# bmorris3/frei

Hardware: AMD Instinct MI355X
Metric: lambda-bin*layer flux updates/sec at 60 layers x 500k lambda (higher is better)
Workload: dtype f64; 1 GPU; C3/C4: 60 layers x 500000 lambda, 8 species (H2O/CO/CO2/CH4/Na/K + H2-H2/H2-He CIA), 16 T-nodes, 1 step = 1 T-P iteration (emit+absorb); n_layers=60, n_lambda=500000, n_species=8, n_T=16, parallelism=lambda-shard x1

## Files before the change

frei_amd/csrc/frei_device.h:

```cpp
#pragma once
#include <hip/hip_runtime.h>

#include <algorithm>
#include <cstdint>
#include <string>

namespace frei {

constexpr double kH = 6.62607015e-27;
constexpr double kC = 29979245800.0;
constexpr double kHC = kH * kC;
constexpr double kKB = 1.380649e-16;
constexpr double kMP = 1.67262192369e-24;
constexpr double kMbarDefault = 2.4 * kMP;
constexpr double kSigmaSB = 5.6703744191844314e-05;
constexpr double kPi = 3.141592653589793;

constexpr int kEmit = 0;
constexpr int kAbsorb = 1;
constexpr int kBlock = 256;
constexpr int kMaxLayers = 1024;

__host__ __device__ inline int step_layer(int dir, int k, int nL) {
  return dir == kEmit ? k + 1 : nL - 2 - k;
}
__host__ __device__ inline int layer_step(int dir, int i, int nL) {
  const int k = dir == kEmit ? i - 1 : nL - 2 - i;
  return (k >= 0 && k < nL - 1) ? k : -1;
}

struct StepP {
  double iT1, iT2;
  double dm;
  int32_t layer;
  int32_t top;
  int64_t pad;
};

constexpr int kMaxFastS = 8;
struct FastStep {
  double iT1, iT2, dm;
  int32_t layer, top;
  double wlo[kMaxFastS], whi[kMaxFastS], mmr[kMaxFastS];
  int64_t off[kMaxFastS];
};

struct FastStepS {
  double iT1, iT2, dm, wlo, whi;
  int64_t off;
  int32_t layer, top;
  double mmr[kMaxFastS];
};
static_assert(sizeof(FastStepS) % sizeof(double) == 0, "FastStepS is staged as doubles");

struct TermP {
  const double* row[4];
  double w[4];
  double mmr;
  double x1, dx;
  int32_t nrow;
  int32_t pad;
};

struct SpecMeta {
  const double* tab;
  int64_t n_lam;
  int32_t n_p, n_T;
  int32_t t_off;
  int32_t one_T;
};

struct PMeta {
  int32_t p_lo, p_hi;
  double wp_lo, wp_hi;
  double x1, dx;
  int32_t oob;
  int32_t pad;
};

__host__ __device__ inline void bracket(const double* g, int n, double x, int& i, double& y,
                                        int& oob) {
  int lo = 0, hi = n;
  while (lo < hi) {
    const int mid = (lo + hi) >> 1;
    if (g[mid] < x) lo = mid + 1; else hi = mid;
  }
  i = lo - 1;
  if (i < 0) i = 0;
  if (i > n - 2) i = n - 2;
  y = (x - g[i]) / (g[i + 1] - g[i]);
  oob = (x < g[0] || x > g[n - 1]) ? 1 : 0;
}

__host__ __device__ inline TermP make_term(const SpecMeta& sm, const PMeta& pm,
                                           const double* tnodes, const int32_t* tperm,
                                           double mmr, double T, int fast) {
  TermP t;
  for (int r = 0; r < 4; ++r) { t.row[r] = sm.tab; t.w[r] = 0.0; }
  t.mmr = mmr;
  t.x1 = 0.0;
  t.dx = 1.0;
  t.nrow = 0;
  t.pad = 0;
  const int64_t rowlen = sm.n_lam;
  if (sm.one_T) {
    if (pm.oob) return t;
    const int tp = tperm[sm.t_off];
    t.row[0] = sm.tab + ((int64_t)pm.p_lo * sm.n_T + tp) * rowlen;
    t.row[1] = sm.tab + ((int64_t)pm.p_hi * sm.n_T + tp) * rowlen;
    t.x1 = pm.x1;
    t.dx = pm.dx;
    t.nrow = -1;
    return t;
  }
  int it, oobT;
  double yt;
  bracket(tnodes + sm.t_off, sm.n_T, T, it, yt, oobT);
  if (pm.oob || oobT) {
    if (fast) t.nrow = 2;
    return t;
  }
  const int tlo = tperm[sm.t_off + it], thi = tperm[sm.t_off + it + 1];
  const int pr[2] = {pm.p_lo, pm.p_hi};
  const double wp[2] = {pm.wp_lo, pm.wp_hi};
  const int tr[2] = {tlo, thi};
  const double wt[2] = {1.0 - yt, yt};
  int n = 0;
  for (int a = 0; a < 2; ++a) {
    if (wp[a] == 0.0) continue;
    for (int b = 0; b < 2; ++b) {
      t.row[n] = sm.tab + ((int64_t)pr[a] * sm.n_T + tr[b]) * rowlen;
      t.w[n] = (1.0 * wp[a]) * wt[b];
      ++n;
    }
  }
  t.nrow = n;
  return t;
}

__host__ __device__ inline void fast_term(const SpecMeta& sm, const PMeta& pm,
                                          const double* tnodes, double T, int64_t& off,
                                          double& wlo, double& whi) {
  int it, oobT;
  double yt;
  bracket(tnodes + sm.t_off, sm.n_T, T, it, yt, oobT);
  off = 0;
  wlo = whi = 0.0;
  if (pm.oob || oobT) return;
  const int prow = (pm.wp_lo != 0.0) ? pm.p_lo : pm.p_hi;
  const double wp = (pm.wp_lo != 0.0) ? pm.wp_lo : pm.wp_hi;
  off = ((int64_t)prow * sm.n_T + it) * sm.n_lam;
  wlo = (1.0 * wp) * (1.0 - yt);
  whi = (1.0 * wp) * yt;
}

struct AtmStride {
  int64_t layers;
  int64_t steps;
  int64_t fb;
  int64_t hist;
  int64_t flux;
  int64_t tab;
  int64_t part;
  int64_t ftoa;
  const double* g;
};

struct ChemArgs {
  const double* tab;
  const double* T;
  const int32_t* pj;
  const double* pz;
  int n_T, n_p;
  const int32_t* atm_tab;
  int64_t tab_stride;
};

__host__ __device__ inline void chem_bracket(const double* g, int n, double x, int& i,
                                             double& y) {
  i = 0;
  y = 0.0;
  if (n < 2) return;
  const double xc = x < g[0] ? g[0] : (x > g[n - 1] ? g[n - 1] : x);
  int lo = 0, hi = n - 2;
  while (lo < hi) {
    const int mid = (lo + hi + 1) >> 1;
    if (g[mid] <= xc) lo = mid; else hi = mid - 1;
  }
  i = lo;
  y = (xc - g[i]) / (g[i + 1] - g[i]);
}

__host__ __device__ inline double chem_mmr_at(const ChemArgs& c, int s, int j, double z,
                                              double T) {
  int it;
  double y;
  chem_bracket(c.T, c.n_T, T, it, y);
  const double* v = c.tab + ((int64_t)s * c.n_T + it) * c.n_p;
  auto row = [&](const double* r) { return c.n_p > 1 ? r[j] * (1.0 - z) + r[j + 1] * z : r[0]; };
  const double a = row(v);
  return c.n_T > 1 ? a * (1.0 - y) + row(v + c.n_p) * y : a;
}

struct SetupArgs {
  ChemArgs chem;
  int n_layers, n_species, fast;
  int n_tnodes;
  double* T;
  const double* p;
  double p_top2, g;
  const SpecMeta* spec;
  const PMeta* pmeta;
  const double* tnodes;
  const int32_t* tperm;
  const double* mmr;
  StepP* steps;
  TermP* terms;
  FastStep* fsteps;
  FastStepS* ssteps;
  int shared;
  AtmStride bs;
  int32_t* kvalid;
  int64_t kpitch;
};

struct FastArgs {
  int64_t n_lam;
  int64_t pitch;
  int n_steps, force;
  int live_only;
  const double *c1, *hcl, *sig, *wtr, *ftoa;
  const double* tab[kMaxFastS];
  const FastStep* steps;
  const FastStepS* ssteps;
  double* F_up;
  double* F_down;
  double* dtaus;
  double* part;
  const int* conv;
  AtmStride bs;
  int n_atm;
  int red_rows;
  int unit_mmr;
  int rec_on;
  SetupArgs rec;
  int min_lds;
  const unsigned long long* ch_epoch;
  unsigned long long ch_val;
  int ch_can_conv;
  long long ch_timeout;
  int* ch_err;
  double* poison;
  const double* ktab[kMaxFastS];
  const double* kmmr;
  int kS, kNL;
  double* tail_part;
};
constexpr unsigned long long kPoisonT = 0xFFF4F4F4F4F4F4F4ull;

struct SweepArgs {
  int64_t n_lam;
  int n_steps, n_species, force;
  int live_only;
  const double *c1, *hcl, *sig, *wtr, *ftoa;
  const StepP* steps;
  const TermP* terms;
  double* F_up;
  double* F_down;
  double* dtaus;
  double* part;
  const int* conv;
};

struct P2PPush {
  double* const* peers;
  int nranks, rank;
  int64_t n;
  uint64_t seq;
};
struct P2PWait {
  const double* mbox;
  int nranks;
  int64_t n;
  uint64_t seq;
  int64_t timeout_ticks;
  int* err;
  unsigned long long* wait_ticks;
};
__host__ __device__ inline int64_t mbox_val(int par, int r, int R, int64_t n) {
// ... 159 lines not shown
```

frei_amd/csrc/frei_kernels.hip:

```cpp
#include <type_traits>
#include <unordered_map>

#include "frei_device.h"
#include "frei_math.h"

namespace frei {

template <auto V, auto... Rest, typename F>
static void pick(decltype(V) v, F&& f) {
  if constexpr (sizeof...(Rest) == 0) {
    f(std::integral_constant<decltype(V), V>{});
  } else {
    if (v == V) f(std::integral_constant<decltype(V), V>{});
    else pick<Rest...>(v, f);
  }
}

static void lds_optin(const void* kernel, size_t lds) {
  if (lds <= 65536) return;
  static std::unordered_map<const void*, size_t> optin;
  size_t& have = optin[kernel];
  if (lds > have) {
    (void)hipFuncSetAttribute(kernel, hipFuncAttributeMaxDynamicSharedMemorySize, (int)lds);
    have = lds;
// ... 1653 lines not shown
    for (int i = 0; i < G; ++i) stn[i] = stale(0, i);
    PT_STAMP(DIR, bx, wv, -1, 0);
    for (int ph = 0; ph <= nph; ++ph) {
      if (ph >= 1) {
        const int q = ph - 1;
        double stc[G];
#pragma unroll
        for (int i = 0; i < G; ++i) stc[i] = stn[i];
#pragma unroll
        for (int i = 0; i < G; ++i) stn[i] = stale(ph, i);
        double rv[G][kPipeNV];
        read_ring(q, rv);
#pragma unroll
        for (int i = 0; i < G; ++i) step(q, i, stc[i], rv[i]);
      }
      PT_STAMP(DIR, bx, wv, ph, 0);
      __syncthreads();
      PT_STAMP(DIR, bx, wv, ph, 1);
    }
  }
  TRACE_MARK(2);
  if constexpr (!TL) {
    __syncthreads();
    for (int idx = tid; idx < ns * 4; idx += 256 * NC) {
      double s = red[idx];
      for (int w = 1; w < NC; ++w) s += red[(int64_t)w * ns * 4 + idx];
      part[part_at(idx, bx, nbx, ns * 4)] = s;
    }
  }
  TRACE_PUT(CH ? 50 + NC : TL ? 60 + NC : 20 + NC);
}

template <int DIR, int NC, int M, int PF>
__global__ __launch_bounds__(256 * NC) __attribute__((amdgpu_waves_per_eu(4)))
void sweep_pipe_kernel(FastArgs a, const FastStepS* __restrict__ ss, double* __restrict__ Fu,
                       double* __restrict__ Fd, double* __restrict__ part,
                       double* __restrict__ dtaus) {
  extern __shared__ double lds[];
  sweep_pipe_body<DIR, NC, M, PF, false>(a, ss, Fu, Fd, part, dtaus, lds, blockIdx.x, gridDim.x);
}

void launch_sweep_pipe(int dir, int NC, int PF, const FastArgs& a, int nblocks,
                       hipStream_t st) {
  pick<kEmit, kAbsorb>(dir, [&](auto D) {
    pick<4, 2, 1>(NC, [&](auto nc) {
      pick<2, 1>(PF, [&](auto pf) {
        launch_lds(sweep_pipe_kernel<D(), nc(), 2, pf()>,
                   dim3(nblocks, a.n_atm > 1 ? a.n_atm : 1), dim3(256 * nc()),
                   pipe_lds_bytes(nc(), 2, a.n_steps), st, a, a.ssteps, a.F_up, a.F_down, a.part,
                   a.dtaus);
      });
    });
  });
}

size_t pipe_lds_bytes(int NC, int M, int ns) {
  return (size_t)pipe_lds_doubles(NC, M, ns) * sizeof(double);
}

__device__ __forceinline__ void p2p_push_values(const P2PPush& p, int64_t idx, const double* v,
                                                int nv) {
  const int par = (int)(p.seq & 1);
  for (int r = 0; r < p.nranks; ++r) {
    uint64_t* dst = reinterpret_cast<uint64_t*>(p.peers[r] + mbox_val(par, p.rank, p.nranks, p.n));
    for (int k = 0; k < nv; ++k)
      __hip_atomic_store(dst + idx + k, __builtin_bit_cast(uint64_t, v[k]), __ATOMIC_RELAXED,
                         __HIP_MEMORY_SCOPE_SYSTEM);
  }
  __builtin_amdgcn_fence(__ATOMIC_RELEASE, "");
  asm volatile("s_waitcnt vmcnt(0)" ::: "memory");
  for (int r = 0; r < p.nranks; ++r) {
    uint64_t* fl = reinterpret_cast<uint64_t*>(p.peers[r]) + mbox_flag(par, p.rank, p.nranks, p.n);
    for (int k = 0; k < nv; ++k)
      __hip_atomic_store(fl + idx + k, p.seq, __ATOMIC_RELAXED, __HIP_MEMORY_SCOPE_SYSTEM);
  }
}

__device__ __forceinline__ void p2p_wait(const P2PWait& w, int r, int64_t idx, long long t0) {
  const int par = (int)(w.seq & 1);
  const uint64_t* fl =
      reinterpret_cast<const uint64_t*>(w.mbox) + mbox_flag(par, r, w.nranks, w.n) + idx;
  while (__hip_atomic_load(fl, __ATOMIC_RELAXED, __HIP_MEMORY_SCOPE_SYSTEM) != w.seq) {
    if (wall_clock64() - t0 > w.timeout_ticks ||
        __hip_atomic_load(w.err, __ATOMIC_RELAXED, __HIP_MEMORY_SCOPE_AGENT)) {
      __hip_atomic_store(w.err, 1, __ATOMIC_RELAXED, __HIP_MEMORY_SCOPE_AGENT);
      break;
    }
    __builtin_amdgcn_s_sleep(1);
  }
}

__device__ __forceinline__ void p2p_acquire() { __builtin_amdgcn_fence(__ATOMIC_ACQUIRE, ""); }

__device__ __forceinline__ double p2p_value(const P2PWait& w, int r, int64_t idx) {
  const int par = (int)(w.seq & 1);
  const uint64_t* vp =
      reinterpret_cast<const uint64_t*>(w.mbox + mbox_val(par, r, w.nranks, w.n)) + idx;
  return __builtin_bit_cast(double,
                            __hip_atomic_load(vp, __ATOMIC_RELAXED, __HIP_MEMORY_SCOPE_SYSTEM));
}

__global__ void p2p_handshake_kernel(P2PPush push, P2PWait wait) {
  if (threadIdx.x != 0) return;
  const double one = 1.0;
  p2p_push_values(push, 0, &one, 1);
  const long long t0 = wall_clock64();
  for (int r = 0; r < wait.nranks; ++r) p2p_wait(wait, r, 0, t0);
  p2p_acquire();
}

void launch_p2p_handshake(const P2PPush& push, const P2PWait& wait, hipStream_t st) {
  hipLaunchKernelGGL(p2p_handshake_kernel, dim3(1), dim3(64), 0, st, push, wait);
}

constexpr int kRedThreads = 256;
constexpr int kRedWaves = kRedThreads / 64;

__global__ __launch_bounds__(kRedThreads) void reduce_kernel(const double* __restrict__ part,
                                                     int nblocks, double* __restrict__ Fb,
                                                     const int* conv, int force,
                                                     int64_t part_stride, int64_t fb_stride,
                                                     P2PPush push) {
  part += blockIdx.y * part_stride;
  Fb += blockIdx.y * fb_stride;
  conv += blockIdx.y;
  if (!force && *conv) return;
  __shared__ double sh[kRedWaves];
  const int ns4 = gridDim.x;
  double acc = 0.0;
  for (int b = threadIdx.x; b < nblocks; b += kRedThreads)
    acc += part[part_at(blockIdx.x, b, nblocks, ns4)];
  acc = butterfly_sum(acc, threadIdx.x & 63);
  if ((threadIdx.x & 63) == 0) sh[threadIdx.x >> 6] = acc;
  __syncthreads();
  if (threadIdx.x == 0) {
    double v = sh[0];
    for (int w = 1; w < kRedWaves; ++w) v += sh[w];
    if (push.peers) p2p_push_values(push, blockIdx.x, &v, 1);
    else Fb[blockIdx.x] = v;
  }
}

__global__ void log_ratio_kernel(const double* __restrict__ p, double p_top2, int nL,
                                 double* __restrict__ lnp) {
  const int l = blockIdx.x * blockDim.x + threadIdx.x;
  if (l < nL) lnp[l] = log(p[l] / (l == nL - 1 ? p_top2 : p[l + 1]));
}

void launch_log_ratio(const double* p, double p_top2, int nL, double* lnp, hipStream_t st) {
  hipLaunchKernelGGL(log_ratio_kernel, dim3((nL + 255) / 256), dim3(256), 0, st, p, p_top2,
                     nL, lnp);
}

__device__ __forceinline__ void step_s_core(const SetupArgs& u, const double* T, const double* P,
                                            const double* tnodes, const SpecMeta& sm,
                                            const PMeta& pm, int dir, int k, FastStepS& f) {
  const int nL = u.n_layers;
  const int i = step_layer(dir, k, nL);
  const int top = (dir == kEmit && i == nL - 1) ? 1 : 0;
  f.layer = i;
  f.top = top;
  f.iT1 = 1.0 / T[i];
  f.iT2 = top ? f.iT1 : 1.0 / T[i + 1];
  const double p2 = top ? u.p_top2 : P[i + 1];
  f.dm = (P[i] - p2) / u.g;
  int64_t off;
  double wlo, whi;
  fast_term(sm, pm, tnodes, T[i], off, wlo, whi);
  f.off = off;
  f.wlo = wlo;
  f.whi = whi;
}
__device__ void setup_sweep(const SetupArgs& u, const double* T, const double* P,
                            const double* tnodes, const SpecMeta* spec, const PMeta* pmeta,
                            const double* mmr, int dir, int kb, int ke, int tid, int nthr,
                            int mstride, int mbase) {
  const int nS = u.n_species;
  const int nL = u.n_layers;
  auto MI = [&](int s, int i) { return (int64_t)s * mstride + (i - mbase); };
  auto MMR = [&](int s, int i) {
    return u.chem.tab ? chem_mmr_at(u.chem, s, u.chem.pj[i], u.chem.pz[i], T[i])
                      : mmr[MI(s, i)];
  };
  if (u.fast && u.shared) {
    for (int k = kb + tid; k < ke; k += nthr) {
      const int i = step_layer(dir, k, nL);
      FastStepS* f = u.ssteps + k;
      step_s_core(u, T, P, tnodes, spec[0], pmeta[MI(0, i)], dir, k, *f);
      for (int s = 0; s < kMaxFastS; ++s) f->mmr[s] = s < nS ? MMR(s, i) : 0.0;
    }
    return;
  }
  if (u.fast) {
    for (int k = kb + tid; k < ke; k += nthr) {
      const int i = step_layer(dir, k, nL);
      FastStep* f = u.fsteps + k;
      const int top = (dir == kEmit && i == nL - 1) ? 1 : 0;
      f->layer = i;
      f->top = top;
      f->iT1 = 1.0 / T[i];
      f->iT2 = top ? f->iT1 : 1.0 / T[i + 1];
      const double p2 = top ? u.p_top2 : P[i + 1];
      f->dm = (P[i] - p2) / u.g;
    }
    for (int idx = tid; idx < (ke - kb) * kMaxFastS; idx += nthr) {
      const int k = kb + idx / kMaxFastS, s = idx % kMaxFastS;
      FastStep* f = u.fsteps + k;
      if (s >= nS) {
        if (!(u.kvalid && s == 1)) f->off[s] = 0;
        f->wlo[s] = f->whi[s] = f->mmr[s] = 0.0;
        continue;
      }
      const int i = step_layer(dir, k, nL);
      int64_t off;
      double wlo, whi;
      fast_term(spec[s], pmeta[MI(s, i)], tnodes, T[i], off, wlo, whi);
      f->off[s] = off;
      f->wlo[s] = wlo;
      f->whi[s] = whi;
      f->mmr[s] = MMR(s, i);
      if (u.kvalid && s == 0) {
        int64_t mask = 0;
        if (wlo != 0.0 || whi != 0.0) {
          const int64_t r = off / u.kpitch;
          mask = (u.kvalid[r] ? 0 : 1) | (u.kvalid[r + 1] ? 0 : 2);
        }
        f->off[1] = mask;
      }
    }
    return;
  }
  for (int k = kb + tid; k < ke; k += nthr) {
    const int i = step_layer(dir, k, nL);
    StepP sp;
    sp.layer = i;
    sp.top = (dir == kEmit && i == nL - 1) ? 1 : 0;
    sp.iT1 = 1.0 / T[i];
    sp.iT2 = sp.top ? sp.iT1 : 1.0 / T[i + 1];
    const double p2 = sp.top ? u.p_top2 : P[i + 1];
    sp.dm = (P[i] - p2) / u.g;
    sp.pad = 0;
    u.steps[k] = sp;
  }
  for (int idx = tid; idx < (ke - kb) * nS; idx += nthr) {
    const int k = kb + idx / nS, s = idx % nS;
    const int i = step_layer(dir, k, nL);
    u.terms[(int64_t)k * nS + s] = make_term(spec[s], pmeta[MI(s, i)], tnodes, u.tperm, MMR(s, i),
                             T[i], u.fast);
  }
}

__device__ inline void atm_view(SetupArgs& u, int m) {
  u.T += m * u.bs.layers;
  u.steps += m * u.bs.steps;
  u.fsteps += m * u.bs.steps;
  u.ssteps += m * u.bs.steps;
  if (u.bs.g) u.g = u.bs.g[m];
  if (u.chem.atm_tab) u.chem.tab += u.chem.atm_tab[m] * u.chem.tab_stride;
}

__device__ inline void atm_view(UpdateArgs& a, int m) {
  atm_view(a.su, m);
  const AtmStride& b = a.su.bs;
  a.Fb += m * b.fb;
  a.Tb += m * b.layers;
  a.Ta += m * b.layers;
  a.hist += m * b.hist;
  a.flips += m * b.layers;
  a.prev_sign += m * b.layers;
  a.ndiff += m * b.layers;
  a.iter += m;
  a.conv += m;
  if (a.dT_out) a.dT_out += m * b.layers;
  if (a.bol_out) a.bol_out += m * b.layers * 4;
}

__global__ void setup_kernel(SetupArgs u, int dir) {
  atm_view(u, blockIdx.x);
  setup_sweep(u, u.T, u.p, u.tnodes, u.spec, u.pmeta, u.mmr, dir, 0, u.n_layers - 1,
              threadIdx.x, blockDim.x, u.n_layers, 0);
}

struct LayerPre {
  double dz, cp, dF_conv, dt_rad, dt_conv, rho0, cp0;
  bool conv;
};

__device__ __forceinline__ LayerPre layer_pre(double T1, double T2, double p1, double p2,
                                              double lnp, double g, double m_bar,
                                              double alpha) {
  LayerPre r;
  r.dz = (kKB * T1) / (m_bar * g) * lnp;
  r.cp = (2 + 5) / (2 * m_bar) * kKB;
  const double rho = ((p1 - p2) / g) / r.dz;
  const double dg = (T1 - T2) / r.dz - g / r.cp;
  r.conv = dg > 0;
  r.dF_conv = 0.0;
  r.dt_conv = 0.0;
  if (r.conv) {
    const double lmix = alpha * kKB * T1 / (m_bar * g);
    r.dF_conv = rho * r.cp * (lmix * lmix) * sqrt(g / T1) * pow(dg, 1.5);
    r.dt_conv = sqrt(T1 / g / dg);
  }
  r.dt_rad = r.cp * p1 / kSigmaSB / g / pow(T1, 3.0);
  const double m0 = kMbarDefault;
  const double dz0 = (kKB * T1) / (m0 * g) * lnp;
  r.rho0 = ((p1 - p2) / g) / dz0;
  r.cp0 = (2 + 5) / (2 * m0) * kKB;
  return r;
}

__device__ __forceinline__ double layer_dT_post(const double* Fb, const LayerPre& r) {
  const double dF_rad = (Fb[0] - Fb[1]) - (Fb[2] - Fb[3]);
  const double div = (dF_rad + r.dF_conv) / r.dz;
  const double x = div * r.dz;
  const double f = (x != 0) ? 1e5 / pow(fabs(x), 0.9) : 1.0;
  const double dt = r.conv ? f * fmin(r.dt_rad, r.dt_conv) : f * r.dt_rad;
  return 1 / r.rho0 / r.cp0 * div * dt;
}

__device__ double layer_dT(const double* Fb, double T1, double T2, double p1, double p2,
                           double lnp, double g, double m_bar, double alpha) {
  return layer_dT_post(Fb, layer_pre(T1, T2, p1, p2, lnp, g, m_bar, alpha));
}


__global__ __launch_bounds__(256) void update_kernel(UpdateArgs a) {
  atm_view(a, blockIdx.x);
  if (!a.force && *a.conv) return;
  extern __shared__ __attribute__((aligned(16))) double sh[];
  __shared__ int all_conv;
  const int nL = a.su.n_layers;
  const int ns = nL - 1;
  const int dir = a.dir;
  const int S = a.su.n_species;
  const int ntn = a.su.n_tnodes;
  double* sT = sh;
  double* sdT = sT + nL;
  double* sP = sdT + nL;
  double* sTb = sP + nL;
  double* sTa = sTb + nL;
  double* sLn = sTa + nL;
  double* sTn = sLn + nL;
  double* sFb = sTn + ntn;
  int* sFl = reinterpret_cast<int*>(sFb + ns * 4);
  int* sPv = sFl + nL;
  int* sNd = sPv + nL;
  const bool meta = a.meta_in_lds;
  char* mb = reinterpret_cast<char*>(sh) + (((reinterpret_cast<char*>(sNd + nL) -
                                              reinterpret_cast<char*>(sh)) + 15) & ~15);
  PMeta* sPm = reinterpret_cast<PMeta*>(mb);
  double* sMm = reinterpret_cast<double*>(sPm + (meta ? S * nL : 0));
  SpecMeta* sSp = reinterpret_cast<SpecMeta*>(sMm + (meta ? S * nL : 0));
  if (threadIdx.x == 0) all_conv = 1;
  for (int l = threadIdx.x; l < nL; l += blockDim.x) {
    sT[l] = a.su.T[l];
    sdT[l] = 0.0;
    sP[l] = a.su.p[l];
    sLn[l] = a.lnp[l];
    if (a.track) {
      sTb[l] = a.Tb[l];
      sTa[l] = a.Ta[l];
      sFl[l] = a.flips[l];
      sPv[l] = a.prev_sign[l];
      sNd[l] = a.ndiff[l];
    }
  }
  for (int q = threadIdx.x; q < ntn; q += blockDim.x) sTn[q] = a.su.tnodes[q];
  if (a.p2p.mbox) {
    const long long t0 = wall_clock64();
    for (int q = threadIdx.x; q < ns * 4; q += blockDim.x)
      for (int r = 0; r < a.p2p.nranks; ++r) p2p_wait(a.p2p, r, q, t0);
    p2p_acquire();
    for (int q = threadIdx.x; q < ns * 4; q += blockDim.x) {
      double v = p2p_value(a.p2p, 0, q);
      for (int r = 1; r < a.p2p.nranks; ++r) v += p2p_value(a.p2p, r, q);
      sFb[q] = v;
    }
    __syncthreads();
    if (threadIdx.x == 0 && a.p2p.wait_ticks)
      atomicAdd(a.p2p.wait_ticks, (unsigned long long)(wall_clock64() - t0));
  } else {
    for (int q = threadIdx.x; q < ns * 4; q += blockDim.x) {
      double v = a.Fb[q];
      for (int r = 1; r < a.nranks; ++r) v += a.Fb[(int64_t)r * ns * 4 + q];
      sFb[q] = v;
    }
  }
  if (meta) {
    for (int q = threadIdx.x; q < S * nL; q += blockDim.x) {
      sPm[q] = a.su.pmeta[q];
      sMm[q] = a.su.mmr[q];
    }
    for (int q = threadIdx.x; q < S; q += blockDim.x) sSp[q] = a.su.spec[q];
  }
  __syncthreads();
  for (int k = threadIdx.x; k < ns; k += blockDim.x) {
    const int i = step_layer(dir, k, nL);
    const double* Fb = sFb + k * 4;
    if (a.bol_out)
      for (int q = 0; q < 4; ++q) a.bol_out[(int64_t)i * 4 + q] = Fb[q];
    const bool top = (dir == kEmit && i == nL - 1);
    const double T1 = sT[i];
    const double T2 = top ? T1 : sT[i + 1];
    const double p2 = top ? a.su.p_top2 : sP[i + 1];
    sdT[i] = layer_dT(Fb, T1, T2, sP[i], p2, sLn[i], a.su.g, a.m_bar, a.alpha);
  }
  __syncthreads();
  const int it = *a.iter;
  for (int l = threadIdx.x; l < nL; l += blockDim.x) {
    const double dT = sdT[l];
    const double Tnew = sT[l] - dT;
    if (a.dT_out) a.dT_out[l] = dT;
    if (a.track) {
      if (dir == kEmit) {
        a.Tb[l] = Tnew;
      } else {
        const double Tb = sTb[l];
        if (it < a.hist_cap) {
          a.hist[((int64_t)it * 2 + 0) * nL + l] = Tb;
          a.hist[((int64_t)it * 2 + 1) * nL + l] = Tnew;
        }
        int flips = sFl[l], prev = sPv[l], nd = sNd[l];
        const double d0 = Tb - sTa[l], d1 = Tnew - Tb;
        for (int q = (it > 0 ? 0 : 1); q < 2; ++q) {
          const double d = q == 0 ? d0 : d1;
          const int sgn = (d > 0) - (d < 0);
          if (nd > 0 && sgn != prev) ++flips;
          prev = sgn;
          ++nd;
        }
        a.flips[l] = flips;
        a.prev_sign[l] = prev;
        a.ndiff[l] = nd;
        a.Ta[l] = Tnew;
        const bool c = (flips > a.n_zero_crossings) || (fabs(dT) < a.convergence_dT);
        if (!c) atomicAnd(&all_conv, 0);
      }
    }
    a.su.T[l] = Tnew;
    sT[l] = Tnew;
  }
  __syncthreads();
  if (threadIdx.x == 0 && a.track && dir == kAbsorb) {
    *a.iter = it + 1;
    if (all_conv && a.stop_on_conv) *a.conv = 1;
  }
  if (a.next_dir >= 0)
    setup_sweep(a.su, sT, sP, sTn, meta ? sSp : a.su.spec, meta ? sPm : a.su.pmeta,
                meta ? sMm : a.su.mmr, a.next_dir, 0, ns, threadIdx.x, blockDim.x, nL, 0);
}

__device__ __forceinline__ void publish_T(const UpdateArgs& a, int l, double T, int conv0,
                                          bool c) {
  if (a.epoch) {
    __hip_atomic_store(reinterpret_cast<unsigned long long*>(a.T_out) + l,
                       __builtin_bit_cast(unsigned long long, T), __ATOMIC_RELAXED,
                       __HIP_MEMORY_SCOPE_AGENT);
    __hip_atomic_store(a.epoch + l,
                       (a.epoch_val << 2) | (conv0 ? 2ull : 0ull) | (c ? 1ull : 0ull),
                       __ATOMIC_RELAXED, __HIP_MEMORY_SCOPE_AGENT);
  } else {
    a.T_out[l] = T;
  }
}
__device__ __forceinline__ void update_arrive(const UpdateArgs& a, int nU, int it, bool nc1) {
  if (!(a.track && a.dir == kAbsorb)) return;
  const unsigned old = __hip_atomic_fetch_add(a.done, 1u + (nc1 ? 65536u : 0u),
                                              __ATOMIC_RELAXED, __HIP_MEMORY_SCOPE_AGENT);
  if ((old & 0xffffu) != (unsigned)nU - 1) return;
  const unsigned nc = (old >> 16) + (nc1 ? 1u : 0u);
  *a.iter = it + 1;
  if (nc == 0 && a.stop_on_conv) *a.conv = 1;
  __hip_atomic_store(a.done, 0u, __ATOMIC_RELAXED, __HIP_MEMORY_SCOPE_AGENT);
}

template <int U = 1>
__device__ void update_fused_body(const UpdateArgs& a, int lr, int nU, int tid, int h,
                                  double* sh) {
  TRACE_DECL;
  const int nL = a.su.n_layers;
  const bool on = lr < nL;
  const int l = on ? lr : nL - 1;
  const int dir = a.dir;
  const double* Tin = a.su.T;
  double* sTn = sh;
  double* sP = sTn + nL;
  double* sNodes = sP + nL;
  __shared__ double wsum_[4][kRedWaves][8];
  __shared__ double tot_[4][8];
  __shared__ PMeta sPm_[4][kMaxFastS];
  __shared__ SpecMeta sSp_[4][kMaxFastS];
  __shared__ double sMm_[4][kMaxFastS];
  auto& wsum = wsum_[h];
  double* tot = tot_[h];
  PMeta* sPm = sPm_[h];
  SpecMeta* sSp = sSp_[h];
  double* sMm = sMm_[h];
  const int k0 = layer_step(dir, l, nL);
  const int k1 = l + 1 < nL ? layer_step(dir, l + 1, nL) : -1;
  const int kn = a.next_dir >= 0 ? layer_step(a.next_dir, l, nL) : -1;
  const int S = a.su.n_species;
  const bool stage = S <= kMaxFastS;
  const int conv = *a.conv;
  const int it = *a.iter;
  const int ntn = a.su.n_tnodes;
  const double rNode = a.su.tnodes[tid < ntn ? tid : ntn - 1];
  const int li = min(l + (tid & 1), nL - 1);
  const int li1 = min(li + 1, nL - 1);
  const int kd = (tid & 1) ? k1 : k0;
  const bool top = (dir == kEmit && li == nL - 1);
  const double T1 = Tin[li];
  const double rT2 = Tin[li1];
  const double p1 = a.su.p[li];
  const double rp2 = a.su.p[li1];
  const double lnp = a.lnp[li];
  const double Tb = a.Tb[l], Ta = a.Ta[l];
  int flips = a.flips[l], prev = a.prev_sign[l], nd = a.ndiff[l];
  const int sm = min(max(tid - 64, 0), S - 1);
  const PMeta rPm = a.su.pmeta[(int64_t)sm * nL + l];
  const SpecMeta rSp = a.su.spec[sm];
  const double rMm = a.su.mmr[(int64_t)sm * nL + l];
  const double T2 = top ? T1 : rT2;
  const double p2 = top ? a.su.p_top2 : rp2;
  const double Tl = T1;
  LayerPre pre{};
  if (tid < 2 && kd >= 0) pre = layer_pre(T1, T2, p1, p2, lnp, a.su.g, a.m_bar, a.alpha);
  if (k0 >= 0 || k1 >= 0) {
    const double* pj[8];
    for (int j = 0; j < 8; ++j) {
      const int k = (j < 4) ? (k0 >= 0 ? k0 : k1) : (k1 >= 0 ? k1 : k0);
      pj[j] = a.part + part_at(k * 4 + (j & 3), 0, a.nblocks, 4 * (nL - 1));
    }
    const int64_t bs = part_at(0, 1, a.nblocks, 4 * (nL - 1));
    double acc[8];
    for (int j = 0; j < 8; ++j) acc[j] = 0.0;
    constexpr int kU = U;
    const int nb = a.nblocks;
    if constexpr (U == 1) {
#pragma unroll 2
      for (int b = tid; b < nb; b += kRedThreads)
        for (int j = 0; j < 8; ++j) acc[j] += pj[j][b * bs];
    } else
    for (int b0 = tid; b0 < nb; b0 += kU * kRedThreads) {
      double v[kU][8];
#pragma unroll
      for (int u = 0; u < kU; ++u) {
        const int b = min(b0 + u * kRedThreads, nb - 1);
#pragma unroll
        for (int j = 0; j < 8; ++j) v[u][j] = pj[j][b * bs];
      }
#pragma unroll
      for (int u = 0; u < kU; ++u)
        if (b0 + u * kRedThreads < nb)
#pragma unroll
          for (int j = 0; j < 8; ++j) acc[j] += v[u][j];
    }
    for (int j = 0; j < 8; ++j)
      acc[j] = butterfly_sum(acc[j], tid & 63);
    if ((tid & 63) == 0)
      for (int j = 0; j < 8; ++j) wsum[tid >> 6][j] = acc[j];
  }
  if (!a.force && conv) {
    if (tid == 0 && on) publish_T(a, l, Tl, conv, true);
    return;
  }
  if (tid < ntn) sNodes[tid] = rNode;
  for (int q = tid + kRedThreads; q < ntn; q += kRedThreads) sNodes[q] = a.su.tnodes[q];
  if (kn >= 0) {
    const int s = tid - 64;
    if (stage && s >= 0 && s < S) {
      sPm[s] = rPm;
      sSp[s] = rSp;
      sMm[s] = rMm;
    }
    if (tid < 2 && l + tid < nL) sP[l + tid] = p1;
    if (tid == 1 && l + 1 < nL) sTn[l + 1] = T1;
  }
  __syncthreads();
  TRACE_MARK(1);
  if (tid < 8) {
    double t = wsum[0][tid];
    for (int w = 1; w < kRedWaves; ++w) t += wsum[w][tid];
    tot[tid] = t;
  }
  __syncthreads();
  const long long t0 = wall_clock64();
  if (a.p2p.mbox && tid == 64 && k0 >= 0 && on)
    p2p_push_values(a.push, (int64_t)k0 * 4, tot, 4);
  if (tid < 64) {
    double v = 0.0;
    const int k = tid < 4 ? k0 : k1;
    if (tid < 8 && k >= 0) {
      v = tot[tid];
      if (a.p2p.mbox) {
        const double own = v;
        const int64_t idx = (int64_t)k * 4 + (tid & 3);
        for (int r = 0; r < a.p2p.nranks; ++r)
          if (r != a.push.rank) p2p_wait(a.p2p, r, idx, t0);
        p2p_acquire();
        for (int r = 0; r < a.p2p.nranks; ++r) {
          const double x = (r == a.push.rank) ? own : p2p_value(a.p2p, r, idx);
          v = (r == 0) ? x : v + x;
        }
      }
    }
    const int base = (tid & 1) * 4;
    double F[4];
    for (int q = 0; q < 4; ++q) F[q] = __shfl(v, base + q, 64);
    if (tid < 4 && k0 >= 0 && a.bol_out && on) a.bol_out[(int64_t)l * 4 + tid] = v;
    if (tid == 0 && lr == 0 && a.p2p.mbox && a.p2p.wait_ticks)
      atomicAdd(a.p2p.wait_ticks, (unsigned long long)(wall_clock64() - t0));
    double d = 0.0;
    if (tid < 2 && kd >= 0) {
      d = layer_dT_post(F, pre);
      sTn[li] = T1 - d;
    }
    if (tid == 0 && on) {
      const double dT = d;
      const double Tnew = Tl - dT;
      if (a.dT_out) a.dT_out[l] = dT;
      bool c = true;
      if (a.track) {
        if (dir == kEmit) {
          a.Tb[l] = Tnew;
        } else {
          if (it < a.hist_cap) {
            a.hist[((int64_t)it * 2 + 0) * nL + l] = Tb;
            a.hist[((int64_t)it * 2 + 1) * nL + l] = Tnew;
          }
          const double d0 = Tb - Ta, d1 = Tnew - Tb;
          for (int q = (it > 0 ? 0 : 1); q < 2; ++q) {
            const double dd = q == 0 ? d0 : d1;
            const int sgn = (dd > 0) - (dd < 0);
            if (nd > 0 && sgn != prev) ++flips;
            prev = sgn;
            ++nd;
          }
          a.flips[l] = flips;
          a.prev_sign[l] = prev;
          a.ndiff[l] = nd;
          a.Ta[l] = Tnew;
          c = (flips > a.n_zero_crossings) || (fabs(dT) < a.convergence_dT);
        }
      }
      publish_T(a, l, Tnew, conv, c);
      if (kd < 0) sTn[l] = Tnew;
      update_arrive(a, nU, it, !c);
    }
  }
  TRACE_MARK(2);
  __syncthreads();
  if (a.su.kvalid && tid == 64 && on && k0 >= 0) {
    int64_t off;
    double wlo, whi;
    fast_term(rSp, rPm, sNodes, Tl, off, wlo, whi);
    if (wlo != 0.0 || whi != 0.0) {
      const int64_t r = off / a.su.kpitch;
      a.su.kvalid[r] = 1;
      a.su.kvalid[r + 1] = 1;
    }
  }
  if (kn >= 0 && tid >= 64 && on) {
    if (stage)
      setup_sweep(a.su, sTn, sP, sNodes, sSp, sPm, sMm, a.next_dir, kn, kn + 1, tid - 64,
                  kRedThreads - 64, 1, l);
    else
      setup_sweep(a.su, sTn, sP, sNodes, a.su.spec, a.su.pmeta, a.su.mmr, a.next_dir, kn,
                  kn + 1, tid - 64, kRedThreads - 64, nL, 0);
  }
  TRACE_PUT(30);
}

__device__ __forceinline__ void update_shadow(const UpdateArgs& a) {
  if (!a.force && *a.conv) return;
  __syncthreads();
  __syncthreads();
  __syncthreads();
}

__global__ __launch_bounds__(kRedThreads) void update_fused_kernel(UpdateArgs a) {
  extern __shared__ __attribute__((aligned(16))) double sh[];
  update_fused_body<8>(a, blockIdx.x, gridDim.x, threadIdx.x, 0, sh);
}

template <int DIR, int Q, int NW>
__global__ __launch_bounds__(64 * NW) void sweep_chain_kernel(
    FastArgs a, UpdateArgs u, const FastStepS* __restrict__ ss, double* __restrict__ Fu,
    double* __restrict__ Fd, double* __restrict__ part, double* __restrict__ dtaus) {
  static_assert(kRedThreads == 256, "update halves of 256 threads");
  extern __shared__ double red[];
  const int nL = u.su.n_layers;
  constexpr int kHalves = NW / 4;
  const int nU = (nL + kHalves - 1) / kHalves;
  if ((int)blockIdx.x < nU) {
    const int h = threadIdx.x >> 8;
    update_fused_body(u, blockIdx.x * kHalves + h, nL, threadIdx.x & 255, h,
                      red + (int64_t)h * (2 * nL + u.su.n_tnodes));
    return;
  }
  sweep_group_body<DIR, Q, NW, true>(a, ss, Fu, Fd, part, dtaus, red, blockIdx.x - nU,
                                     gridDim.x - nU);
}

template <int DIR, int PF>
__global__ __launch_bounds__(1024) __attribute__((amdgpu_waves_per_eu(4)))
void sweep_pipe_chain_kernel(FastArgs a, UpdateArgs u, const FastStepS* __restrict__ ss,
                             double* __restrict__ Fu, double* __restrict__ Fd,
                             double* __restrict__ part, double* __restrict__ dtaus) {
  static_assert(kRedThreads == 256, "update parts of 256 threads");
  extern __shared__ double lds[];
  const int nL = u.su.n_layers;
  if ((int)blockIdx.x < nL) {
    if (threadIdx.x < 256) update_fused_body(u, blockIdx.x, nL, threadIdx.x, 0, lds);
    else update_shadow(u);
    return;
  }
  sweep_pipe_body<DIR, 4, 2, PF, true>(a, ss, Fu, Fd, part, dtaus, lds, blockIdx.x - nL,
                                       gridDim.x - nL);
}

void launch_sweep_pipe_chain(int dir, int PF, const FastArgs& a, const UpdateArgs& u,
                             int nblocks, hipStream_t st) {
  const int nL = u.su.n_layers;
  const size_t shm = std::max(pipe_lds_bytes(4, 2, a.n_steps),
                              (size_t)(2 * nL + u.su.n_tnodes) * sizeof(double));
  pick<kEmit, kAbsorb>(dir, [&](auto D) {
    pick<2, 1>(PF, [&](auto pf) {
      launch_lds(sweep_pipe_chain_kernel<D(), pf()>, dim3(nL + nblocks), dim3(1024), shm, st, a,
                 u, a.ssteps, a.F_up, a.F_down, a.part, a.dtaus);
    });
  });
}

struct TailIn {
  double *T, *p, *Tb, *Ta, *mmr, *nodes;
  int *flips, *prev, *nd;
  PMeta* pm;
  LayerPre* pre;
};
__host__ __device__ inline size_t tail_in_bytes(int nL, int ntn) {
  return (size_t)nL * (sizeof(PMeta) + sizeof(LayerPre)) + (size_t)(5 * nL + ntn) * sizeof(double) +
         (size_t)3 * nL * sizeof(int);
}
__device__ __forceinline__ TailIn tail_in_layout(double* lds, int nL, int ntn) {
  TailIn t;
  t.pre = reinterpret_cast<LayerPre*>(lds);
  t.pm = reinterpret_cast<PMeta*>(t.pre + nL);
  double* d = reinterpret_cast<double*>(t.pm + nL);
  t.T = d;
  t.p = d + nL;
  t.Tb = d + 2 * nL;
  t.Ta = d + 3 * nL;
  t.mmr = d + 4 * nL;
  t.nodes = d + 5 * nL;
  int* q = reinterpret_cast<int*>(t.nodes + ntn);
  t.flips = q;
  t.prev = q + nL;
  t.nd = q + 2 * nL;
  return t;
}

#ifdef FREI_TRACE
__shared__ unsigned long long g_tail_done[4];
__shared__ unsigned g_tail_pass[4];
#endif
__device__ __forceinline__ void tail_update_slot(const UpdateArgs& a, int lr, int tid, int h,
                                                 double (&wsum)[kRedWaves][8],
                                                 const TailIn& in, int conv, int it) {
  TRACE_DECL;
  const int nL = a.su.n_layers;
  const bool on = lr < nL;
  const int l = on ? lr : nL - 1;
  const int dir = a.dir;
  const int k0 = layer_step(dir, l, nL);
  const int k1 = l + 1 < nL ? layer_step(dir, l + 1, nL) : -1;
  const bool skip = !a.force && conv;
  const bool sums = !skip && (k0 >= 0 || k1 >= 0);
  const int nb = a.nblocks;
  if (sums) {
    const double* pj[8];
    for (int j = 0; j < 8; ++j) {
      const int k = (j < 4) ? (k0 >= 0 ? k0 : k1) : (k1 >= 0 ? k1 : k0);
      pj[j] = a.part + (int64_t)(k * 4 + (j & 3)) * nb;
    }
    const int b = min(tid, nb - 1);
    unsigned long long x[8];
    auto load_all = [&]() {
      bool m = false;
#pragma unroll
      for (int j = 0; j < 8; ++j) {
        x[j] = __hip_atomic_load((const gu64*)(pj[j] + b), __ATOMIC_RELAXED, __HIP_MEMORY_SCOPE_AGENT);
        m |= x[j] == kPoisonT;
      }
      return m;
    };
    bool miss = load_all();
#ifdef FREI_TRACE
    int passes = 1;
#endif
    if (__any(miss)) {
      const long long t0 = wall_clock64();
      do {
        __builtin_amdgcn_s_sleep(1);
        miss = load_all();
#ifdef FREI_TRACE
        ++passes;
#endif
        const int e = __hip_atomic_load(a.poll_err, __ATOMIC_RELAXED, __HIP_MEMORY_SCOPE_AGENT);
        if (__any(miss) && (e || wall_clock64() - t0 > a.poll_timeout)) {
          if (!e) __hip_atomic_store(a.poll_err, 3, __ATOMIC_RELAXED, __HIP_MEMORY_SCOPE_AGENT);
          break;
        }
      } while (__any(miss));
    }
#ifdef FREI_TRACE
    atomicMax(&g_tail_done[h], (unsigned long long)wall_clock64());
    atomicMax(&g_tail_pass[h], (unsigned)passes);
#endif
    double acc[8];
    for (int j = 0; j < 8; ++j) acc[j] = tid < nb ? 0.0 + __builtin_bit_cast(double, x[j]) : 0.0;
    for (int j = 0; j < 8; ++j) acc[j] = butterfly_sum(acc[j], tid & 63);
    if ((tid & 63) == 0)
      for (int j = 0; j < 8; ++j) wsum[tid >> 6][j] = acc[j];
  }
  __syncthreads();
  TRACE_MARK(2);
#ifdef FREI_TRACE
  if (sums) {
    unsigned long long dm = 0;
    unsigned pm = 0;
    for (int q = 0; q < 4; ++q) dm = max(dm, g_tail_done[q]), pm = max(pm, g_tail_pass[q]);
    tr_[1] = (long long)(dm & ((1ull << 40) - 1)) | ((long long)pm << 40);
  }
  __syncthreads();
  if (tid == 0) g_tail_done[h] = 0, g_tail_pass[h] = 0;
// ... 634 lines not shown
      smm[q] = a.mmr[((int64_t)(m0 + m) * S + s) * a.n_layers + l];
    }
    __syncthreads();
    if (live)
      for (int m = 0; m < nm; ++m) {
        const double* mm = smm + m * S;
        dbl2 acc = mm[0] * v[0];
#pragma unroll
        for (int s = 1; s < S; ++s) acc = acc + mm[s] * v[s];
        *reinterpret_cast<dbl2*>(a.eff + (int64_t)(m0 + m) * a.tab_stride + at) = acc;
      }
  }
}

void launch_contract_batch_valu(const double* const* tabs, int S, const double* mmr,
                                const int32_t* prow, int n_layers, int n_T, int64_t pitch,
                                int n_atm, int64_t tab_stride, double* eff, hipStream_t st) {
  ContractBatchArgs a{};
  for (int s = 0; s < S && s < kMaxFastS; ++s) a.tab[s] = tabs[s];
  a.mmr = mmr;
  a.prow = prow;
  a.eff = eff;
  a.S = S;
  a.n_layers = n_layers;
  a.n_T = n_T;
  a.n_atm = n_atm;
  a.pitch = pitch;
  a.tab_stride = tab_stride;
  const int64_t ncol = (int64_t)n_T * pitch;
  dim3 grid((unsigned)((ncol / 2 + 255) / 256), (unsigned)n_layers);
  switch (S) {
#define K7V(n) case n: hipLaunchKernelGGL(contract_batch_valu_kernel<n>, grid, dim3(256), 0, st, a); break;
    K7V(1) K7V(2) K7V(3) K7V(4) K7V(5) K7V(6) K7V(7)
    default: hipLaunchKernelGGL(contract_batch_valu_kernel<8>, grid, dim3(256), 0, st, a);
#undef K7V
  }
}

void launch_contract_batch(const double* const* tabs, int S, const double* mmr,
                           const int32_t* prow, int n_layers, int n_T, int64_t pitch,
                           int n_atm, int64_t tab_stride, double* eff, hipStream_t st) {
  ContractBatchArgs a{};
  for (int s = 0; s < S && s < kMaxFastS; ++s) a.tab[s] = tabs[s];
  a.mmr = mmr;
  a.prow = prow;
  a.eff = eff;
  a.S = S;
  a.n_layers = n_layers;
  a.n_T = n_T;
  a.n_atm = n_atm;
  a.pitch = pitch;
  a.tab_stride = tab_stride;
  const int64_t ncol = (int64_t)n_T * pitch;
  dim3 grid((unsigned)((ncol + 4 * kK7Cols - 1) / (4 * kK7Cols)), (unsigned)n_layers);
  switch (S) {
#define K7M(n) case n: hipLaunchKernelGGL(contract_batch_kernel<n>, grid, dim3(256), 0, st, a); break;
    K7M(1) K7M(2) K7M(3) K7M(4) K7M(5) K7M(6) K7M(7)
    default: hipLaunchKernelGGL(contract_batch_kernel<8>, grid, dim3(256), 0, st, a);
#undef K7M
  }
}

__global__ void fill_kernel(double* x, int64_t n, double v) {
  for (int64_t idx = (int64_t)blockIdx.x * blockDim.x + threadIdx.x; idx < n;
       idx += (int64_t)gridDim.x * blockDim.x)
    x[idx] = v;
}

void launch_sweep(int dir, const SweepArgs& a, int nblocks, hipStream_t st) {
  const size_t shm = (size_t)(kBlock / 64) * a.n_steps * 4 * sizeof(double);
  pick<kEmit, kAbsorb>(dir, [&](auto D) {
    launch_lds(sweep_kernel<D()>, dim3(nblocks), dim3(kBlock), shm, st, a);
  });
}

void launch_sweep_fast(int dir, int S, int depth, int pf, bool nan_check, bool shared,
                       const FastArgs& a, int nblocks, hipStream_t st) {
  const bool one = S == 1 && !nan_check;
  const bool mm1 = one && a.unit_mmr;
  int PD = depth >= 2 ? 2 : 1, PF = 0;
  if (mm1 && pf > depth && depth >= 2) {
    PD = fast_pd(depth);
    PF = fast_pf_or_0(pf);
  } else if (mm1 && depth == 1 && pf == 2) {
    PF = 2;
  } else if (one && depth >= 4) {
    PD = 4;
  }
  pick<kEmit, kAbsorb>(dir, [&](auto D) {
    pick<true, false>(shared, [&](auto SH) {
      auto go = [&](auto s, auto pd, auto nanchk, auto m1, auto f) {
        const size_t shm = SH() ? lds_steps_bytes(a)
                                : (size_t)red_lds_doubles(a.red_rows, a.n_steps) * sizeof(double);
        launch_lds(sweep_fast_kernel<D(), s(), pd(), nanchk(), SH(), m1(), f() ? f() : pd()>,
                   dim3(nblocks, a.n_atm > 1 ? a.n_atm : 1), dim3(kBlock), with_min_lds(a, shm),
                   st, a, a.steps, a.ssteps, a.F_up, a.F_down, a.part, a.dtaus);
      };
      constexpr std::integral_constant<int, 1> k1{};
      constexpr std::integral_constant<int, 4> k4{};
      constexpr std::integral_constant<int, 0> k0{};
      if (mm1 && PD == 1) {
        pick<2, 0>(PF, [&](auto f) { go(k1, k1, std::false_type{}, std::true_type{}, f); });
      } else if (mm1) {
        pick<4, 2>(PD, [&](auto pd) {
          pick<16, 8, 0>(PF, [&](auto f) { go(k1, pd, std::false_type{}, std::true_type{}, f); });
        });
      } else if (PD == 4) {
        go(k1, k4, std::false_type{}, std::false_type{}, k0);
      } else {
        pick<2, 1>(PD, [&](auto pd) {
          pick<true, false>(nan_check, [&](auto nanchk) {
            pick<1, 2, 3, 4, 5, 6, 7, 8>(S, [&](auto s) {
              go(s, pd, nanchk, std::false_type{}, k0);
            });
          });
        });
      }
    });
  });
}

__global__ void nan_scan_kernel(const double* __restrict__ x, int64_t n, int* flag) {
  int found = 0;
  for (int64_t i = (int64_t)blockIdx.x * blockDim.x + threadIdx.x; i < n;
       i += (int64_t)gridDim.x * blockDim.x)
    found |= isnan(x[i]) ? 1 : 0;
  if (__any(found) && (threadIdx.x & 63) == 0) atomicOr(flag, 1);
}

void launch_nan_scan(const double* x, int64_t n, int* flag, hipStream_t st) {
  hipLaunchKernelGGL(nan_scan_kernel, dim3(2048), dim3(256), 0, st, x, n, flag);
}

void launch_reduce(const double* part, int nblocks, double* Fb, int n_idx, const int* conv,
                   int force, hipStream_t st, int n_atm, int64_t part_stride,
                   int64_t fb_stride, const P2PPush* push) {
  P2PPush p{};
  if (push) p = *push;
  hipLaunchKernelGGL(reduce_kernel, dim3(n_idx, n_atm), dim3(kRedThreads), 0, st, part, nblocks, Fb,
                     conv, force, part_stride, fb_stride, p);
}

void launch_setup(const SetupArgs& u, int dir, hipStream_t st, int n_atm) {
  hipLaunchKernelGGL(setup_kernel, dim3(n_atm), dim3(256), 0, st, u, dir);
}

void launch_update(const UpdateArgs& a, hipStream_t st, int n_atm) {
  const size_t shm = update_lds_bytes(a.su.n_layers, a.su.n_tnodes, a.su.n_species,
                                      a.meta_in_lds != 0);
  hipLaunchKernelGGL(update_kernel, dim3(n_atm), dim3(256), shm, st, a);
}

void launch_update_fused(const UpdateArgs& a, hipStream_t st) {
  const size_t shm = (2 * (size_t)a.su.n_layers + a.su.n_tnodes) * sizeof(double);
  hipLaunchKernelGGL(update_fused_kernel, dim3(a.su.n_layers), dim3(kRedThreads), shm, st, a);
}

void launch_propagate(int64_t n, const double* c1, const double* lk, const double* F1u,
                      const double* F2d, double T1, double T2, const double* dtau,
                      const double* w0, const double* g0, double* F2u, double* F1d,
                      hipStream_t st) {
  const int nb = (int)((n + 255) / 256);
  hipLaunchKernelGGL(propagate_kernel, dim3(nb), dim3(256), 0, st, n, c1, lk, F1u, F2d, T1,
                     T2, dtau, w0, g0, F2u, F1d);
}

void launch_kappa(int64_t n, const TermP* terms, int nS, const double* sig, double* k,
                  hipStream_t st) {
  const int nb = (int)((n + 255) / 256);
  hipLaunchKernelGGL(kappa_kernel, dim3(nb), dim3(256), 0, st, n, terms, nS, sig, k);
}

void launch_gen_table(double* tab, const double* base, const double* fp, const double* fT,
                      int n_p, int n_T, int64_t n_lam, int64_t stride, double lo, double hi,
                      hipStream_t st) {
  hipLaunchKernelGGL(gen_table_kernel, dim3(4096), dim3(256), 0, st, tab, base, fp, fT, n_p,
                     n_T, n_lam, stride, lo, hi);
}

void launch_fill(double* x, int64_t n, double v, hipStream_t st) {
  const int nb = (int)std::min<int64_t>((n + 255) / 256, 4096);
  hipLaunchKernelGGL(fill_kernel, dim3(nb > 0 ? nb : 1), dim3(256), 0, st, x, n, v);
}

}

#ifdef FREI_TRACE
extern "C" int frei_trace_fetch(long long* rec, int n_max, int* n) {
  unsigned cnt = 0;
  if (hipMemcpyFromSymbol(&cnt, HIP_SYMBOL(frei::g_trace_n), sizeof(cnt)) != hipSuccess) return -1;
  const unsigned m = cnt < (unsigned)n_max ? cnt : (unsigned)n_max;
  if (m && hipMemcpyFromSymbol(rec, HIP_SYMBOL(frei::g_trace), m * sizeof(frei::TraceRec)) !=
               hipSuccess)
    return -1;
  *n = (int)cnt;
  const unsigned zero = 0;
  return hipMemcpyToSymbol(HIP_SYMBOL(frei::g_trace_n), &zero, sizeof(zero)) == hipSuccess ? 0 : -1;
}
extern "C" int frei_ptrace_fetch(long long* out, int n_max) {
  const size_t n = sizeof(frei::g_ptrace) / sizeof(long long);
  if ((size_t)n_max < n) return -1;
  return hipMemcpyFromSymbol(out, HIP_SYMBOL(frei::g_ptrace), sizeof(frei::g_ptrace)) == hipSuccess
             ? (int)n
             : -1;
}
#endif
```

Before: 148.8 billion updates/s.

## Stage partial-sum reduction through LDS with vectorized double2 loads in fused update

The fused update kernel's reduction over per-block partial sums now issues double2 vector loads into registers, writes them to a swizzled LDS staging buffer, and then has each thread accumulate contiguous blocks. The first batch of loads is issued early so it overlaps the layer precompute. The goal is to replace many strided scalar global loads with coalesced vector loads and to hide their latency. In exchange the kernel needs 64 KB of extra LDS and more registers, which may lower occupancy. Smaller refactors of the make_term row selection and the next-pressure lookup ride along.

After: 148.8 billion updates/s, median of 2. No clear change (-0.0%).

```diff
diff --git a/frei_amd/csrc/frei_device.h b/frei_amd/csrc/frei_device.h
--- a/frei_amd/csrc/frei_device.h
+++ b/frei_amd/csrc/frei_device.h
@@ -121,20 +121,23 @@
     return t;
   }
   const int tlo = tperm[sm.t_off + it], thi = tperm[sm.t_off + it + 1];
-  const int pr[2] = {pm.p_lo, pm.p_hi};
-  const double wp[2] = {pm.wp_lo, pm.wp_hi};
-  const int tr[2] = {tlo, thi};
-  const double wt[2] = {1.0 - yt, yt};
-  int n = 0;
-  for (int a = 0; a < 2; ++a) {
-    if (wp[a] == 0.0) continue;
-    for (int b = 0; b < 2; ++b) {
-      t.row[n] = sm.tab + ((int64_t)pr[a] * sm.n_T + tr[b]) * rowlen;
-      t.w[n] = (1.0 * wp[a]) * wt[b];
-      ++n;
-    }
-  }
-  t.nrow = n;
+  const double wt_lo = 1.0 - yt, wt_hi = yt;
+  const bool lo = !(pm.wp_lo == 0.0), hi = !(pm.wp_hi == 0.0);
+  const int p0 = lo ? pm.p_lo : pm.p_hi;
+  const double wp0 = lo ? pm.wp_lo : pm.wp_hi;
+  if (lo || hi) {
+    t.row[0] = sm.tab + ((int64_t)p0 * sm.n_T + tlo) * rowlen;
+    t.w[0] = (1.0 * wp0) * wt_lo;
+    t.row[1] = sm.tab + ((int64_t)p0 * sm.n_T + thi) * rowlen;
+    t.w[1] = (1.0 * wp0) * wt_hi;
+  }
+  if (lo && hi) {
+    t.row[2] = sm.tab + ((int64_t)pm.p_hi * sm.n_T + tlo) * rowlen;
+    t.w[2] = (1.0 * pm.wp_hi) * wt_lo;
+    t.row[3] = sm.tab + ((int64_t)pm.p_hi * sm.n_T + thi) * rowlen;
+    t.w[3] = (1.0 * pm.wp_hi) * wt_hi;
+  }
+  t.nrow = 2 * ((lo ? 1 : 0) + (hi ? 1 : 0));
   return t;
 }
 
diff --git a/frei_amd/csrc/frei_kernels.hip b/frei_amd/csrc/frei_kernels.hip
--- a/frei_amd/csrc/frei_kernels.hip
+++ b/frei_amd/csrc/frei_kernels.hip
@@ -1829,6 +1829,11 @@
                      nL, lnp);
 }
 
+__device__ __forceinline__ double next_p(const SetupArgs& u, const double* P, int i, int top) {
+  const double above = P[top ? i : i + 1], p_top2 = u.p_top2;
+  return top ? p_top2 : above;
+}
+
 __device__ __forceinline__ void step_s_core(const SetupArgs& u, const double* T, const double* P,
                                             const double* tnodes, const SpecMeta& sm,
                                             const PMeta& pm, int dir, int k, FastStepS& f) {
@@ -1839,7 +1844,7 @@
   f.top = top;
   f.iT1 = 1.0 / T[i];
   f.iT2 = top ? f.iT1 : 1.0 / T[i + 1];
-  const double p2 = top ? u.p_top2 : P[i + 1];
+  const double p2 = next_p(u, P, i, top);
   f.dm = (P[i] - p2) / u.g;
   int64_t off;
   double wlo, whi;
@@ -1877,7 +1882,7 @@
       f->top = top;
       f->iT1 = 1.0 / T[i];
       f->iT2 = top ? f->iT1 : 1.0 / T[i + 1];
-      const double p2 = top ? u.p_top2 : P[i + 1];
+      const double p2 = next_p(u, P, i, top);
       f->dm = (P[i] - p2) / u.g;
     }
     for (int idx = tid; idx < (ke - kb) * kMaxFastS; idx += nthr) {
@@ -1914,7 +1919,7 @@
     sp.top = (dir == kEmit && i == nL - 1) ? 1 : 0;
     sp.iT1 = 1.0 / T[i];
     sp.iT2 = sp.top ? sp.iT1 : 1.0 / T[i + 1];
-    const double p2 = sp.top ? u.p_top2 : P[i + 1];
+    const double p2 = next_p(u, P, i, sp.top);
     sp.dm = (P[i] - p2) / u.g;
     sp.pad = 0;
     u.steps[k] = sp;
@@ -2152,9 +2157,76 @@
   __hip_atomic_store(a.done, 0u, __ATOMIC_RELAXED, __HIP_MEMORY_SCOPE_AGENT);
 }
 
-template <int U = 1>
+typedef double dbl2s __attribute__((ext_vector_type(2)));
+constexpr int kStageBlocks = 1024;
+constexpr int kStageLoads = kStageBlocks * 4 / kRedThreads;
+constexpr size_t kStageBytes = (size_t)kStageBlocks * 4 * sizeof(dbl2s);
+__device__ __forceinline__ int stage_slot(int b, int s) { return b * 4 + (s ^ ((b >> 2) & 3)); }
+
+constexpr int kStagePer = kRedThreads / 4;
+__device__ __forceinline__ void stage_issue(dbl2s (&v)[2][kStageLoads],
+                                            const double* __restrict__ src, int64_t bs, int nb,
+                                            int tid, int g0) {
+#pragma unroll
+  for (int h = 0; h < 2; ++h)
+    if (g0 + h * kStageBlocks < nb)
+#pragma unroll
+      for (int i = 0; i < kStageLoads; ++i) {
+        const int b = min(g0 + h * kStageBlocks + i * kStagePer + (tid >> 2), nb - 1);
+        v[h][i] = *reinterpret_cast<const dbl2s*>(src + b * bs);
+      }
+}
+__device__ __forceinline__ void sum_partials_staged(dbl2s (&v)[2][kStageLoads],
+                                                    const double* __restrict__ src, int64_t bs,
+                                                    int nb, int tid, dbl2s* stage,
+                                                    double (&acc)[8]) {
+  static_assert(kRedThreads == 256 && kStageBlocks % kRedThreads == 0, "64 blocks per load");
+  constexpr int kPer = kStagePer;
+  const int q = tid & 3;
+  for (int g0 = 0; g0 < nb; g0 += 2 * kStageBlocks) {
+    if (g0 > 0) stage_issue(v, src, bs, nb, tid, g0);
+#pragma unroll
+    for (int h = 0; h < 2; ++h) {
+      const int g = g0 + h * kStageBlocks;
+      if (g < nb) {
+        if (g > 0) __syncthreads();
+#pragma unroll
+        for (int i = 0; i < kStageLoads; ++i)
+          if (g + i * kPer < nb) stage[stage_slot(i * kPer + (tid >> 2), q)] = v[h][i];
+        __syncthreads();
+#pragma unroll
+        for (int u = 0; u < kStageBlocks / kRedThreads; ++u)
+          if (g + u * kRedThreads < nb) {
+            const int bl = u * kRedThreads + tid;
+            dbl2s w[4];
+#pragma unroll
+            for (int s = 0; s < 4; ++s) w[s] = stage[stage_slot(bl, s)];
+            if (g + bl < nb)
+#pragma unroll
+              for (int s = 0; s < 4; ++s) {
+                acc[2 * s] += w[s].x;
+                acc[2 * s + 1] += w[s].y;
+              }
+          }
+      }
+    }
+  }
+}
+
+__device__ __forceinline__ void put_pmeta(PMeta& d, const PMeta& s) {
+  d.p_lo = s.p_lo;
+  d.p_hi = s.p_hi;
+  d.wp_lo = s.wp_lo;
+  d.wp_hi = s.wp_hi;
+  d.x1 = s.x1;
+  d.dx = s.dx;
+  d.oob = s.oob;
+  d.pad = s.pad;
+}
+
+template <bool STAGED = false>
 __device__ void update_fused_body(const UpdateArgs& a, int lr, int nU, int tid, int h,
-                                  double* sh) {
+                                  double* sh, dbl2s* pstage = nullptr) {
   TRACE_DECL;
   const int nL = a.su.n_layers;
   const bool on = lr < nL;
@@ -2201,37 +2273,33 @@
   const double T2 = top ? T1 : rT2;
   const double p2 = top ? a.su.p_top2 : rp2;
   const double Tl = T1;
+  const bool sums = k0 >= 0 || k1 >= 0;
+  const int ka = k0 >= 0 ? k0 : k1, kb = k1 >= 0 ? k1 : k0;
+  const int ns4 = 4 * (nL - 1);
+  const int nb = a.nblocks;
+  const int64_t bs = part_at(0, 1, nb, ns4);
+  const double* src = nullptr;
+  dbl2s sv[STAGED ? 2 : 1][STAGED ? kStageLoads : 1];
+  if constexpr (STAGED)
+    if (sums) {
+      const int q = tid & 3;
+      src = a.part + part_at(((q & 2) ? kb : ka) * 4 + (q & 1) * 2, 0, nb, ns4);
+      stage_issue(sv, src, bs, nb, tid, 0);
+    }
   LayerPre pre{};
   if (tid < 2 && kd >= 0) pre = layer_pre(T1, T2, p1, p2, lnp, a.su.g, a.m_bar, a.alpha);
-  if (k0 >= 0 || k1 >= 0) {
-    const double* pj[8];
-    for (int j = 0; j < 8; ++j) {
-      const int k = (j < 4) ? (k0 >= 0 ? k0 : k1) : (k1 >= 0 ? k1 : k0);
-      pj[j] = a.part + part_at(k * 4 + (j & 3), 0, a.nblocks, 4 * (nL - 1));
-    }
-    const int64_t bs = part_at(0, 1, a.nblocks, 4 * (nL - 1));
+  if (sums) {
     double acc[8];
     for (int j = 0; j < 8; ++j) acc[j] = 0.0;
-    constexpr int kU = U;
-    const int nb = a.nblocks;
-    if constexpr (U == 1) {
+    if constexpr (STAGED) {
+      sum_partials_staged(sv, src, bs, nb, tid, pstage, acc);
+    } else {
+      const double* pj[8];
+      for (int j = 0; j < 8; ++j)
+        pj[j] = a.part + part_at(((j < 4) ? ka : kb) * 4 + (j & 3), 0, nb, ns4);
 #pragma unroll 2
       for (int b = tid; b < nb; b += kRedThreads)
         for (int j = 0; j < 8; ++j) acc[j] += pj[j][b * bs];
-    } else
-    for (int b0 = tid; b0 < nb; b0 += kU * kRedThreads) {
-      double v[kU][8];
-#pragma unroll
-      for (int u = 0; u < kU; ++u) {
-        const int b = min(b0 + u * kRedThreads, nb - 1);
-#pragma unroll
-        for (int j = 0; j < 8; ++j) v[u][j] = pj[j][b * bs];
-      }
-#pragma unroll
-      for (int u = 0; u < kU; ++u)
-        if (b0 + u * kRedThreads < nb)
-#pragma unroll
-          for (int j = 0; j < 8; ++j) acc[j] += v[u][j];
     }
     for (int j = 0; j < 8; ++j)
       acc[j] = butterfly_sum(acc[j], tid & 63);
@@ -2247,7 +2315,7 @@
   if (kn >= 0) {
     const int s = tid - 64;
     if (stage && s >= 0 && s < S) {
-      sPm[s] = rPm;
+      put_pmeta(sPm[s], rPm);
       sSp[s] = rSp;
       sMm[s] = rMm;
     }
@@ -2358,7 +2426,8 @@
 
 __global__ __launch_bounds__(kRedThreads) void update_fused_kernel(UpdateArgs a) {
   extern __shared__ __attribute__((aligned(16))) double sh[];
-  update_fused_body<8>(a, blockIdx.x, gridDim.x, threadIdx.x, 0, sh);
+  update_fused_body<true>(a, blockIdx.x, gridDim.x, threadIdx.x, 0,
+                          sh + kStageBytes / sizeof(double), reinterpret_cast<dbl2s*>(sh));
 }
 
 template <int DIR, int Q, int NW>
@@ -3299,8 +3368,8 @@
 }
 
 void launch_update_fused(const UpdateArgs& a, hipStream_t st) {
-  const size_t shm = (2 * (size_t)a.su.n_layers + a.su.n_tnodes) * sizeof(double);
-  hipLaunchKernelGGL(update_fused_kernel, dim3(a.su.n_layers), dim3(kRedThreads), shm, st, a);
+  const size_t shm = kStageBytes + (2 * (size_t)a.su.n_layers + a.su.n_tnodes) * sizeof(double);
+  launch_lds(update_fused_kernel, dim3(a.su.n_layers), dim3(kRedThreads), shm, st, a);
 }
 
 void launch_propagate(int64_t n, const double* c1, const double* lk, const double* F1u,
```
